# kawshik8/GAN-Image-Captioning

Hardware: AMD Instinct MI355X
Metric: captions/sec (G+D train step) (higher is better)
Workload: dtype bf16; 1 GPU; cfg2: adversarial G+D step, batch 64/GPU, 224x224 images, caption len 20, V=10000, E=H=512, 1-layer LSTM G, CNN-seq D (R=64,F=900), ResNet-50-shaped encoder, --conditional-gan 1; global_batch=64, caption_len=20, image_size=224, vocab=10000, conditional_gan=1, encoder=resnet50, step_impl=fused, parallelism=dp1

## Files before the change

### gan-image-captioning_amd/csrc/decoder.hip

```cpp
#include <stdlib.h>

#include "../../include/gicap.h"
#include "decoder_step.h"
#include "kernels.h"

namespace gic {
namespace {

__device__ __forceinline__ float sigmoidf_(float x) { return 1.f / (1.f + expf(-x)); }

template <typename TA>
__global__ void lstm_pointwise_fwd_kernel(const float* __restrict__ gpre, const float* __restrict__ c_prev,
                                          float* __restrict__ gates, float* __restrict__ c_new,
                                          TA* __restrict__ h_next, long ld_next,
                                          TA* __restrict__ h_up, long ld_up,
                                          TA* __restrict__ h_out, long ld_out,
                                          int B, int H) {
  const int idx = blockIdx.x * blockDim.x + threadIdx.x;
  if (idx >= B * H) return;
  const int b = idx / H, j = idx % H;
  const float* g = gpre + (long)b * 4 * H;
  const float i_ = sigmoidf_(g[j]);
  const float f_ = sigmoidf_(g[H + j]);
  const float g_ = tanhf(g[2 * H + j]);
// ... 240 lines not shown
    *(uint4*)dv[i] = *(const uint4*)(dp + o);
  }
  float s = 0.f;
#pragma unroll
  for (int i = 0; i < NCH; ++i) {
    if (threadIdx.x + 256 * i < nch) {
#pragma unroll
      for (int k = 0; k < VN; ++k) s += to_f32<TA>(pv[i][k]) * to_f32<TA>(dv[i][k]);
    }
  }
  s = block_sum(s, red);
#pragma unroll
  for (int i = 0; i < NCH; ++i) {
    const int c = threadIdx.x + 256 * i;
    if (c < nch) {
      TA ov[VN];
#pragma unroll
      for (int k = 0; k < VN; ++k) ov[k] = from_f32<TA>(temperature * to_f32<TA>(pv[i][k]) * (to_f32<TA>(dv[i][k]) - s));
      *(uint4*)(dl + row * V + (long)c * VN) = *(const uint4*)ov;
    }
  }
}

template <typename TA>
__global__ void build_wcat_kernel(const float* __restrict__ w_ih, const float* __restrict__ w_hh,
                                  const float* __restrict__ b_ih, const float* __restrict__ b_hh,
                                  TA* __restrict__ wcat, float* __restrict__ bsum, int rows, int din, int hid) {
  const long ld = din + hid;
  const long total = (long)rows * ld;
  for (long i = (long)blockIdx.x * blockDim.x + threadIdx.x; i < total; i += (long)gridDim.x * blockDim.x) {
    const long r = i / ld;
    const int c = (int)(i % ld);
    const float v = c < din ? w_ih[r * din + c] : w_hh[r * hid + (c - din)];
    wcat[i] = from_f32<TA>(v);
    if (c == 0) bsum[r] = b_ih[r] + b_hh[r];
  }
}

template <int PB>
__global__ void rollout_join_kernel(const unsigned char* __restrict__ src_xh, unsigned char* __restrict__ dst_xh, long rowbytes,
                                    const float* __restrict__ src_c, float* __restrict__ dst_c, int H, long r0, long r1, int srcB) {
  typedef typename std::conditional<PB == 16, uint4, typename std::conditional<PB == 4, uint32_t, uint16_t>::type>::type piece_t;
  const long pieces = rowbytes / PB;
  const long total = (r1 - r0) * pieces;
  for (long i = (long)blockIdx.x * blockDim.x + threadIdx.x; i < total; i += (long)gridDim.x * blockDim.x) {
    const long r = r0 + i / pieces, p = i % pieces;
    *(piece_t*)(dst_xh + r * rowbytes + p * PB) = *(const piece_t*)(src_xh + (r % srcB) * rowbytes + p * PB);
  }
  const long totc = (r1 - r0) * H;
  for (long i = (long)blockIdx.x * blockDim.x + threadIdx.x; i < totc; i += (long)gridDim.x * blockDim.x) {
    const long r = r0 + i / H;
    dst_c[r * H + i % H] = src_c[(r % srcB) * H + i % H];
  }
}

template <typename TA>
__global__ __launch_bounds__(256) void rollout_pick_kernel(const unsigned long long* __restrict__ rowkey, int64_t* __restrict__ ids, long ids_stride,
                                                           const float* __restrict__ embed, TA* __restrict__ x_next, long ld_x, int rows, int V,
                                                           int E, const int64_t* __restrict__ force_ids, const int32_t* __restrict__ force_len,
// ... 4 lines not shown
  if (force_ids && (!force_len || t < force_len[b])) id = (int)force_ids[(long)b * ids_stride];
  id = id < 0 ? 0 : (id >= V ? V - 1 : id);
  if (lane == 0) ids[(long)b * ids_stride] = id;
  if (x_next)
    for (int e = lane; e < E; e += 64) x_next[(long)b * ld_x + e] = from_f32<TA>(embed[(long)id * E + e]);
}

struct Ctx {
  int B, L, V, E, H, NL, dt;
  int din(int l) const { return l == 0 ? E : H; }
  long ldx(int l) const { return (long)din(l) + H; }
  size_t asz() const { return (size_t)dtype_size(dt); }
};

int check_dims(const gic_decoder_dims* d, Ctx& c) {
  GIC_CHECK_ARG(d, "decoder: null dims");
  GIC_CHECK_ARG(d->B > 0 && d->L > 0 && d->V > 1 && d->E > 0 && d->H > 0, "decoder: bad dims");
  GIC_CHECK_ARG(d->NL >= 1 && d->NL <= GIC_MAX_LAYERS, "decoder: gen_num_layers must be 1..%d", GIC_MAX_LAYERS);
  GIC_CHECK_ARG(d->dtype == DT_F32 || d->dtype == DT_BF16, "decoder: bad dtype");
  c = Ctx{d->B, d->L, d->V, d->E, d->H, d->NL, d->dtype};
  return GIC_OK;
}

int init_slot0(const Ctx& c, const gic_decoder_state* st, const float* features, const gic_decoder_sample_opts* opt, hipStream_t stream) {
  const int B = c.B, E = c.E, H = c.H;
  for (int l = 0; l < c.NL; ++l) {
    if (opt && opt->h0) {
      if (l > 0) GIC_PROPAGATE(fill_zero(st->xh[l], (size_t)B * c.ldx(l) * c.asz(), stream));
      GIC_PROPAGATE(cast2d(opt->h0 + (long)l * B * H, DT_F32, H, (char*)st->xh[l] + (size_t)c.din(l) * c.asz(), c.dt, c.ldx(l), B, H, stream));
    } else {
      GIC_PROPAGATE(fill_zero(st->xh[l], (size_t)B * c.ldx(l) * c.asz(), stream));
    }
    if (opt && opt->c0) GIC_PROPAGATE(cast2d(opt->c0 + (long)l * B * H, DT_F32, H, st->c[l], DT_F32, H, B, H, stream));
    else GIC_PROPAGATE(fill_zero(st->c[l], (size_t)B * H * sizeof(float), stream));
  }
  return cast2d(features, DT_F32, E, st->xh[0], c.dt, c.ldx(0), B, E, stream);
}

template <typename TA>
int sample_fwd_fused(const Ctx& c, const gic_decoder_params* P, const gic_decoder_shadow* S, const gic_decoder_state* st,
                     const float* noise_u, uint64_t seed, float temperature, int pretrain, void* out, int64_t* ids,
                     const gic_decoder_sample_opts* opt, hipStream_t stream) {
  const int B = c.B, L = c.L, V = c.V, H = c.H, NL = c.NL;
  const int nblk = cdiv(V, kVocabTile);
  const long per = (long)L * B * nblk;
  float* part_m = st->part;
  float* part_s = st->part + per;
  unsigned long long* rowkey = (unsigned long long*)(st->part + ((2 * per + 1) & ~1l));
  GIC_PROPAGATE(fill_zero(rowkey, (size_t)L * B * sizeof(unsigned long long), stream));
  const bool keep = !(opt && opt->no_state);
  for (int t = 0; t < L; ++t) {
    for (int l = 0; l < NL; ++l) {
      const long ld = c.ldx(l);
      LstmStepArgs a;
      a.xh_t = (TA*)st->xh[l] + (long)t * B * ld;
      a.xh_next = (TA*)st->xh[l] + (long)(t + 1) * B * ld;
      a.wcat = S->wcat[l]; a.bsum = S->bsum[l];
      a.c_prev = st->c[l] + (long)t * B * H; a.c_new = st->c[l] + (long)(t + 1) * B * H;
      a.gates = keep ? st->gates[l] + (long)t * B * 4 * H : nullptr;
      if (l + 1 < NL) { a.h_up = (TA*)st->xh[l + 1] + (long)t * B * c.ldx(l + 1); a.ld_up = c.ldx(l + 1); }
      if (l + 1 == NL && st->hout) { a.h_out = (TA*)st->hout + (long)t * H; a.ld_out = (long)L * H; }
      a.B = B; a.H = H; a.din = c.din(l); a.ldx = ld;
      if (l == 0 && t > 0) {
        a.gather = 1; a.embed = P->embed; a.V = V;
        a.rowkey = rowkey + (long)(t - 1) * B;
        if (opt && opt->force_ids) { a.force_ids = opt->force_ids; a.force_stride = L; a.force_len = opt->force_len; }
        a.tprev = t - 1;
      }
      GIC_PROPAGATE(lstm_step(a, c.dt, stream));
    }
    VocabStepArgs v;
    const int l = NL - 1;
// ... 1 lines not shown
    v.wout = S->wout; v.bias = P->b_out;
    v.u = noise_u ? noise_u + (long)t * B * V : nullptr;
    v.seed = seed; v.rng_stream = (uint64_t)t; v.temperature = temperature; v.pretrain = pretrain;
    if (opt && opt->dev_scalars) { v.t_dev = &opt->dev_scalars->temperature; v.seed_dev = &opt->dev_scalars->seed[opt->seed_slot]; }
    v.out = out ? (void*)((TA*)out + (long)t * V) : nullptr; v.out_stride = (long)L * V;
    v.part_m = part_m + (long)t * B * nblk; v.part_s = part_s + (long)t * B * nblk; v.rowkey = rowkey + (long)t * B;
    v.nblk = nblk; v.B = B; v.V = V; v.H = H;
    GIC_PROPAGATE(vocab_step(v, c.dt, stream));
  }
  SampleFinishArgs f;
  f.part_m = part_m; f.part_s = part_s; f.rowkey = rowkey; f.nblk = nblk; f.B = B; f.L = L; f.V = V; f.E = c.E;
  f.pretrain = pretrain; f.out = out; f.ids = ids;
  if (opt && opt->force_ids) { f.force_ids = opt->force_ids; f.force_len = opt->force_len; }
  if (keep) { f.embed = P->embed; f.xh0 = st->xh[0]; f.ldx0 = c.ldx(0); }
  return sample_finish(f, c.dt, stream);
}

template <typename TA>
int sample_fwd_t(const Ctx& c, const gic_decoder_params* P, const gic_decoder_shadow* S, const gic_decoder_state* st,
                 const float* features, const float* noise_u, uint64_t seed, float temperature, int pretrain,
                 void* out, int64_t* ids, const gic_decoder_sample_opts* opt, hipStream_t stream) {
  const int B = c.B, L = c.L, V = c.V, E = c.E, H = c.H, NL = c.NL;
  const int pw_grid = cdiv((long)B * H, 256);
  GIC_PROPAGATE(init_slot0(c, st, features, opt, stream));
  if (st->part && B <= decoder_step_max_rows() && !(opt && opt->resume_from) && decoder_step_supported(c.dt, V, E, H, NL))
    return sample_fwd_fused<TA>(c, P, S, st, noise_u, seed, temperature, pretrain, out, ids, opt, stream);
  if (opt && opt->dev_scalars) {
    set_last_error("decoder_sample_fwd: device-resident step scalars need the fused step kernels (state->part, B <= %d, V %% 4 == 0, E, H %% 8 == 0)",
                   decoder_step_max_rows());
    return GIC_ERR_UNSUPPORTED;
  }
  GIC_CHECK_ARG(st->logits && st->gpre, "decoder_sample_fwd: the unfused path needs state->logits and state->gpre");
  const bool keep = !(opt && opt->no_state);
  const int64_t* f_ids = opt ? opt->force_ids : nullptr;
  const int32_t* f_len = opt ? opt->force_len : nullptr;
  const int32_t* act = (opt && opt->resume_from) ? opt->host_active_rows : nullptr;
  if (act) GIC_PROPAGATE(hipMemcpyAsync(ids, f_ids, (size_t)B * L * sizeof(int64_t), hipMemcpyDeviceToDevice, stream) == hipSuccess ? GIC_OK : GIC_ERR_LAUNCH);
  unsigned long long* rowkeys = nullptr;
  if (!out && !pretrain && c.dt == DT_BF16 && V % 4 == 0 && (long)L * 8 <= (long)V * 4 && ((uintptr_t)st->logits & 7) == 0) {
    rowkeys = (unsigned long long*)st->logits;
    GIC_PROPAGATE(fill_zero(rowkeys, (size_t)L * B * sizeof(unsigned long long), stream));
  }

  for (int t = 0; t < L; ++t) {
    const int M = act ? act[t] : B;
    if (act) {
      const int M_prev = t > 0 ? act[t - 1] : 0;
      if (M > M_prev) {
        for (int l = 0; l < NL; ++l) {
          const long rowbytes = c.ldx(l) * (long)c.asz();
          GIC_PROPAGATE(rollout_join((const unsigned char*)opt->resume_from->xh[l] + (size_t)t * opt->resume_B * rowbytes,
                                     (unsigned char*)st->xh[l] + (size_t)t * B * rowbytes, rowbytes,
                                     (const float*)(opt->resume_from->c[l] + (long)t * opt->resume_B * H), st->c[l] + (long)t * B * H, H, M_prev, M,
                                     opt->resume_B, stream));
        }
      }
      if (M == 0) continue;
    }
    const int pw_grid_t = cdiv((long)M * H, 256);
    for (int l = 0; l < NL; ++l) {
      const long ld = c.ldx(l);
      TA* xh_t = (TA*)st->xh[l] + (long)t * B * ld;
      TA* xh_n = (TA*)st->xh[l] + (long)(t + 1) * B * ld;
      GemmDesc g;
      g.A = xh_t; g.lda = ld; g.B = S->wcat[l]; g.ldb = ld; g.C = st->gpre; g.ldc = 4 * H;
// ... 385 lines not shown
int gumbel_softmax_rows(int dt, float* logits, const float* u, uint64_t seed, uint64_t rng_stream, float temperature, int pretrain, void* out,
                        long rows, int V, hipStream_t stream) {
  if (dt == DT_F32)
    hipLaunchKernelGGL((gumbel_softmax_argmax_kernel<float>), dim3((unsigned)rows), dim3(256), 0, stream, logits, u, seed, rng_stream, temperature,
                       pretrain, (float*)out, (long)V, (int64_t*)nullptr, (long)1, (const float*)nullptr, (float*)nullptr, (long)0, V, 0,
                       (const int64_t*)nullptr, (const int32_t*)nullptr, 0);
  else
    hipLaunchKernelGGL((gumbel_softmax_argmax_kernel<bf16_t>), dim3((unsigned)rows), dim3(256), 0, stream, logits, u, seed, rng_stream,
                       temperature, pretrain, (bf16_t*)out, (long)V, (int64_t*)nullptr, (long)1, (const float*)nullptr, (bf16_t*)nullptr, (long)0,
                       V, 0, (const int64_t*)nullptr, (const int32_t*)nullptr, 0);
  GIC_CHECK_LAUNCH("gumbel_softmax (teacher forced)");
  return GIC_OK;
}

namespace {

template <typename TA>
int forward_tf_t(const Ctx& c, const gic_decoder_params* P, const gic_decoder_shadow* S, const gic_decoder_state* st,
                 const float* features, const int64_t* caps, const int32_t* lengths, int Tmax, const float* noise_u, uint64_t seed,
                 float temperature, int pretrain, float* logits_ws, void* out, float* h_n, float* c_n, hipStream_t stream,
                 const gic_sched_sample_opts* ss = nullptr) {
  const int B = c.B, T = c.L, V = c.V, E = c.E, H = c.H, NL = c.NL;
  const int pw_grid = cdiv((long)B * H, 256);
  for (int l = 0; l < NL; ++l) {
    GIC_PROPAGATE(fill_zero(st->xh[l], (size_t)B * c.ldx(l) * c.asz(), stream));
    GIC_PROPAGATE(fill_zero(st->c[l], (size_t)B * H * sizeof(float), stream));
  }
  GIC_PROPAGATE(cast2d(features, DT_F32, E, st->xh[0], c.dt, c.ldx(0), B, E, stream));
  GIC_PROPAGATE(embed_rows_tf(c.dt, P->embed, caps, st->xh[0], c.ldx(0), B, T - 1, E, V, stream));
  const bool ss_fused = ss && ss_fused_logits(c.dt, B, V, E, H, NL);
  if (ss) GIC_PROPAGATE(ss_tail(caps, ss->inputs, ss->replaced, B, T - 1, Tmax - 1, stream));
  for (int t = 0; t < Tmax; ++t) {
    for (int l = 0; l < NL; ++l) {
      const long ld = c.ldx(l);
      TA* xh_t = (TA*)st->xh[l] + (long)t * B * ld;
      TA* xh_n = (TA*)st->xh[l] + (long)(t + 1) * B * ld;
      GemmDesc g;
      g.A = xh_t; g.lda = ld; g.B = S->wcat[l]; g.ldb = ld; g.C = st->gpre; g.ldc = 4 * H;
      g.M = B; g.N = 4 * H; g.K = (int)ld; g.in_dtype = c.dt; g.out_dtype = DT_F32; g.bias = S->bsum[l];
      g.no_split = ss != nullptr;
      GIC_PROPAGATE(gemm(g, stream));
      TA* h_up = (l + 1 < NL) ? (TA*)st->xh[l + 1] + (long)t * B * c.ldx(l + 1) : nullptr;
      TA* h_out = (l + 1 == NL) ? (TA*)st->hout + (long)t * H : nullptr;
      hipLaunchKernelGGL((lstm_pointwise_tf_kernel<TA>), dim3(pw_grid), dim3(256), 0, stream, (const float*)st->gpre,
                         (const float*)(st->c[l] + (long)t * B * H), (const TA*)(xh_t + c.din(l)), ld,
                         st->c[l] + (long)(t + 1) * B * H, xh_n + c.din(l), ld, h_up, h_up ? c.ldx(l + 1) : 0, h_out, (long)Tmax * H,
                         lengths, t, B, H, st->gates[l] ? st->gates[l] + (long)t * B * 4 * H : nullptr);
      GIC_CHECK_LAUNCH("lstm_pointwise_tf");
    }
    if (ss) {
      GIC_PROPAGATE(ss_step_logits(c.dt, st->hout, t, Tmax, S->wout, P->b_out, logits_ws, B, V, H, ss_fused, stream));
// ... 140 lines not shown
}

int gic_decoder_bwd_ws_bytes(const gic_decoder_dims* dims, uint64_t* out) {
  Ctx c;
  GIC_PROPAGATE(check_dims(dims, c));
  GIC_CHECK_ARG(out, "decoder_bwd_ws_bytes: null out");
  const uint64_t B = c.B, L = c.L, H = c.H, a = c.asz();
  out[0] = B * L * (uint64_t)c.V * a;
  out[1] = B * L * H * 4;
  for (int l = 0; l < GIC_MAX_LAYERS; ++l) {
    const bool on = l < c.NL;
    out[2 + l] = on ? L * B * 4 * H * a : 0;
    out[2 + GIC_MAX_LAYERS + l] = on ? (L + 1) * B * (uint64_t)c.ldx(l) * 4 : 0;
    out[2 + 2 * GIC_MAX_LAYERS + l] = on ? B * H * 4 : 0;
  }
  return GIC_OK;
}

int gic_decoder_prepare(const gic_decoder_dims* dims, const gic_decoder_params* P, const gic_decoder_shadow* S, void* stream_) {
  Ctx c;
  GIC_PROPAGATE(check_dims(dims, c));
  GIC_CHECK_ARG(P && S, "decoder_prepare: null struct");
  hipStream_t stream = (hipStream_t)stream_;
  for (int l = 0; l < c.NL; ++l) {
    GIC_CHECK_ARG(P->w_ih[l] && P->w_hh[l] && P->b_ih[l] && P->b_hh[l] && S->wcat[l] && S->bsum[l], "decoder_prepare: null layer %d", l);
    const long total = (long)4 * c.H * c.ldx(l);
    const int grid = (int)((total + 255) / 256 > 2048 ? 2048 : (total + 255) / 256);
    if (c.dt == DT_F32)
      hipLaunchKernelGGL((build_wcat_kernel<float>), dim3(grid), dim3(256), 0, stream, P->w_ih[l], P->w_hh[l], P->b_ih[l],
                         P->b_hh[l], (float*)S->wcat[l], S->bsum[l], 4 * c.H, c.din(l), c.H);
    else
      hipLaunchKernelGGL((build_wcat_kernel<bf16_t>), dim3(grid), dim3(256), 0, stream, P->w_ih[l], P->w_hh[l], P->b_ih[l],
                         P->b_hh[l], (bf16_t*)S->wcat[l], S->bsum[l], 4 * c.H, c.din(l), c.H);
    GIC_CHECK_LAUNCH("build_wcat");
    if (S->wcat_t[l]) GIC_PROPAGATE(transpose2d(S->wcat[l], S->wcat_t[l], c.dt, 4 * c.H, c.ldx(l), stream));
  }
  GIC_CHECK_ARG(P->w_out && S->wout, "decoder_prepare: null w_out");
  if ((const void*)S->wout != (const void*)P->w_out)
    GIC_PROPAGATE(cast2d(P->w_out, DT_F32, c.H, S->wout, c.dt, c.H, c.V, c.H, stream));
  return GIC_OK;
}

int gic_decoder_sample_fwd(const gic_decoder_dims* dims, const gic_decoder_params* P, const gic_decoder_shadow* S,
                           const gic_decoder_state* st, const float* features, const float* noise_u, uint64_t seed,
                           float temperature, int pretrain, void* out, int64_t* ids, const gic_decoder_sample_opts* opt,
                           void* stream) {
  Ctx c;
  GIC_PROPAGATE(check_dims(dims, c));
  GIC_CHECK_ARG(P && S && st && features && ids, "decoder_sample_fwd: null argument");
  const bool keep = !(opt && opt->no_state);
  GIC_CHECK_ARG(!keep || (st->hout && out), "decoder_sample_fwd: out / state->hout may be NULL only for a stateless roll-out (opts->no_state)");
  GIC_CHECK_ARG(!(opt && opt->force_len && !opt->force_ids), "decoder_sample_fwd: force_len without force_ids");
  GIC_CHECK_ARG(!(opt && opt->dev_scalars) || (opt->seed_slot >= 0 && opt->seed_slot < GIC_STEP_SEEDS), "decoder_sample_fwd: seed_slot out of range");
  if (opt && opt->resume_from) {
    GIC_CHECK_ARG(opt->force_ids && opt->force_len && opt->host_active_rows && opt->resume_B > 0 && opt->no_state,
                  "decoder_sample_fwd: resumed roll-outs need force_ids, force_len, host_active_rows, resume_B and no_state");
    for (int l = 0; l < c.NL; ++l) GIC_CHECK_ARG(opt->resume_from->xh[l] && opt->resume_from->c[l], "decoder_sample_fwd: resume_from lacks layer %d state", l);
    for (int t = 0; t < c.L; ++t)
      GIC_CHECK_ARG(opt->host_active_rows[t] >= (t ? opt->host_active_rows[t - 1] : 0) && opt->host_active_rows[t] <= c.B,
                    "decoder_sample_fwd: host_active_rows must be non-decreasing and <= B");
    GIC_CHECK_ARG(opt->host_active_rows[0] == 0, "decoder_sample_fwd: resumed rows have a prefix of at least one token");
  }
  for (int l = 0; l < c.NL; ++l)
// ... 31 lines not shown
```

### gan-image-captioning_amd/csrc/disc.hip

```cpp
#include <stdlib.h>
#include "../../include/gicap.h"
#include "kernels.h"
#include "gemm_device.h"

namespace gic {
namespace {

constexpr int kMaxTaps = 32;
constexpr int kOutDim = 100;
constexpr int kOutPad = 104;

struct ConvMeta {
  int nconv, F, Fp, s;
  int fsize[GIC_MAX_CONVS], nfilt[GIC_MAX_CONVS], foff[GIC_MAX_CONVS];
  const float* w[GIC_MAX_CONVS];
  const float* b[GIC_MAX_CONVS];
  float* dw[GIC_MAX_CONVS];
  float* db[GIC_MAX_CONVS];
};

__device__ __forceinline__ int conv_of(const ConvMeta& cm, int col) {
  int k = 0;
  while (k + 1 < cm.nconv && col >= cm.foff[k + 1]) ++k;
  return k;
// ... 877 lines not shown
  out[5] = MR * Fp * a;
  out[6] = MR * kOutDim * 4;
  return GIC_OK;
}

int gic_disc_bwd_ws_bytes(const gic_disc_dims* dims, uint64_t* out) {
  DCtx c;
  GIC_PROPAGATE(make_ctx(dims, nullptr, nullptr, c));
  GIC_CHECK_ARG(out, "disc_bwd_ws_bytes: null out");
  const uint64_t a = dtype_size(c.dt), MR = c.rowsBR, Fp = c.Fp;
  out[0] = MR * kOutPad * a;
  out[1] = MR * Fp * a;
  out[2] = MR * Fp * 4;
  out[3] = MR * Fp * 4;
  out[4] = (uint64_t)c.rowsBL * c.De * a;
  return GIC_OK;
}

int gic_disc_prepare(const gic_disc_dims* dims, const gic_disc_params* P, const gic_disc_shadow* S, void* stream_) {
  DCtx c;
  GIC_PROPAGATE(make_ctx(dims, P, nullptr, c));
  GIC_CHECK_ARG(P && S && P->emb && P->hw_w && P->f2o_w && S->emb && S->hw_w && S->f2o_w, "disc_prepare: null pointer");
  hipStream_t stream = (hipStream_t)stream_;
  if ((const void*)S->emb != (const void*)P->emb)
    GIC_PROPAGATE(cast2d(P->emb, DT_F32, c.V, S->emb, c.dt, c.V, c.De, c.V, stream));
  const size_t a = dtype_size(c.dt);
  GIC_PROPAGATE(fill_zero(S->hw_w, (size_t)c.Fp * c.Fp * a, stream));
  GIC_PROPAGATE(cast2d(P->hw_w, DT_F32, c.F, S->hw_w, c.dt, c.Fp, c.F, c.F, stream));
  if (S->hw_w_t) GIC_PROPAGATE(transpose2d(S->hw_w, S->hw_w_t, c.dt, c.Fp, c.Fp, stream));
  GIC_PROPAGATE(fill_zero(S->f2o_w, (size_t)kOutPad * c.Fp * a, stream));
  GIC_PROPAGATE(cast2d(P->f2o_w, DT_F32, c.F, S->f2o_w, c.dt, c.Fp, kOutDim, c.F, stream));
  return GIC_OK;
}

int gic_disc_fwd(const gic_disc_dims* dims, const gic_disc_params* P, const gic_disc_shadow* S, const gic_disc_state* st,
                 const void* inp_soft, int64_t ld_inp, const int64_t* inp_ids, int train, const uint8_t* keep_mask,
                 uint64_t seed, float* logits, const gic_step_scalars* dev_scalars, int seed_slot, void* stream) {
  DCtx c;
  GIC_CHECK_ARG(!dev_scalars || (seed_slot >= 0 && seed_slot < GIC_STEP_SEEDS), "disc_fwd: seed_slot out of range");
  const uint64_t* seed_dev = dev_scalars ? &dev_scalars->seed[seed_slot] : nullptr;
  GIC_PROPAGATE(make_ctx(dims, P, nullptr, c));
  GIC_CHECK_ARG(P && S && st && logits, "disc_fwd: null argument");
  GIC_CHECK_ARG((inp_soft != nullptr) != (inp_ids != nullptr), "disc_fwd: pass exactly one of inp_soft / inp_ids");
  GIC_CHECK_ARG(!inp_soft || ld_inp >= c.V, "disc_fwd: ld_inp < V");
  GIC_CHECK_ARG(st->emb && st->pooled && st->ydrop && st->feat && (!train || (st->keep && st->argmax && st->hpre)), "disc_fwd: null state buffer");
  GIC_CHECK_ARG(P->emb && P->hw_b && P->f2o_b && P->o2l_w && P->o2l_b && S->emb && S->hw_w && S->f2o_w, "disc_fwd: null parameter");
  if (c.dt == DT_F32)
    return disc_fwd_t<float>(c, P, S, st, inp_soft, ld_inp, inp_ids, train, keep_mask, seed, seed_dev, logits, (hipStream_t)stream);
  return disc_fwd_t<bf16_t>(c, P, S, st, inp_soft, ld_inp, inp_ids, train, keep_mask, seed, seed_dev, logits, (hipStream_t)stream);
}

int gic_disc_fwd_redrop(const gic_disc_dims* dims, const gic_disc_params* P, const gic_disc_shadow* S, const gic_disc_state* src,
                        const gic_disc_state* dst, int train, const uint8_t* keep_mask, uint64_t seed, float* logits,
                        const gic_step_scalars* dev_scalars, int seed_slot, void* stream) {
  DCtx c;
// ... 50 lines not shown
```

### gan-image-captioning_amd/csrc/kernels.h

```cpp
#pragma once
#include "common.h"
#include "gemm.h"

struct gic_sched_sample_opts;

namespace gic {

int cast2d(const void* src, int src_dtype, long lds, void* dst, int dst_dtype, long ldd, long rows, long cols,
           hipStream_t stream);
int colsum(const void* A, int dtype, long lda, long rows, long cols, float* out, float* out2, int accumulate,
           hipStream_t stream, float* scratch = nullptr, long scratch_floats = 0);
int embedding_fwd(const float* weight, const int64_t* ids, float* out, long n, int V, int E, hipStream_t stream);
int embedding_bwd(const float* d_out, const int64_t* ids, float* d_weight, long n, int V, int E, int zero_first,
                  hipStream_t stream);
int fill_zero(void* p, size_t bytes, hipStream_t stream);
int transpose2d(const void* src, void* dst, int dtype, long rows, long cols, hipStream_t stream);

int decoder_output_bwd(int dt, int B, int L, int V, int H, const void* probs, const void* d_out, float temperature, const float* t_dev, int pretrain,
                       void* dlogits_ws, const void* wout, const void* hout, float* dhout, float* d_wout, float* d_bout, hipStream_t stream);
int lstm_pointwise_fwd(int dt, const float* gpre, const float* c_prev, float* c_new, void* h_next, long ld_next, void* h_up, long ld_up,
                       int rows, int H, hipStream_t stream);
int rollout_join(const unsigned char* src_xh, unsigned char* dst_xh, long rowbytes, const float* src_c, float* dst_c, int H, long r0, long r1,
                 int srcB, hipStream_t stream);
int rollout_pick(int dt, const unsigned long long* rowkey, int64_t* ids, long ids_stride, const float* embed, void* x_next, long ld_x, int rows,
                 int V, int E, const int64_t* force_ids, const int32_t* force_len, int t, hipStream_t stream);
int rollout_argmax(int dt, float* logits, const float* u, uint64_t seed, uint64_t rng_stream, float temperature, int pretrain, void* out,
                   long out_stride, int64_t* ids, long ids_stride, const float* embed, void* x_next, long ld_x, int rows, int V, int E,
                   const int64_t* force_ids, const int32_t* force_len, int t, hipStream_t stream);
int det_mode();
int det_scatter(const void* src, int dt, long ld, long row_off, const int64_t* ids, int B, long s_b, long s_t, long n, float* dst,
                long d_id, long d_e, int E, int V, hipStream_t stream);
int embed_rows_tf(int dt, const float* embed, const int64_t* caps, void* xh0, long ld, int B, int Tm1, int E, int V, hipStream_t stream);
int zero_past_length(float* dhout, const int32_t* lengths, int B, int Tmax, int H, hipStream_t stream);
int gumbel_softmax_rows(int dt, float* logits, const float* u, uint64_t seed, uint64_t rng_stream, float temperature, int pretrain, void* out,
                        long rows, int V, hipStream_t stream);
int embed_scatter_time(const float* dx, long ld, const int64_t* ids, float* d_embed, int B, int L, int E, int V, hipStream_t stream, long ids_stride = 0);

struct SsPickArgs {
  const float* logits = nullptr; long ld_logits = 0;
// ... 24 lines not shown
```

### gan-image-captioning_amd/csrc/util.hip

```cpp
#include <stdarg.h>
#include <stdio.h>

#include "../../include/gicap.h"
#include "kernels.h"

namespace gic {

static thread_local char g_last_error[512] = "";

void set_last_error(const char* fmt, ...) {
  va_list ap;
  va_start(ap, fmt);
  vsnprintf(g_last_error, sizeof(g_last_error), fmt, ap);
  va_end(ap);
}

static thread_local bool g_route_only = false;
static thread_local char g_route[kRouteLen] = "";
bool route_only() { return g_route_only; }
char* route_line() { return g_route; }

namespace {

template <typename TA>
// ... 119 lines not shown

__global__ void embedding_fwd_kernel(const float* __restrict__ w, const int64_t* __restrict__ ids, float* __restrict__ out,
                                     long n, int V, int E) {
  const long total = n * E;
  for (long i = (long)blockIdx.x * blockDim.x + threadIdx.x; i < total; i += (long)gridDim.x * blockDim.x) {
    const long r = i / E;
    const int e = (int)(i % E);
    long id = ids[r];
    id = id < 0 ? 0 : (id >= V ? V - 1 : id);
    out[i] = w[id * E + e];
  }
}

__global__ void embedding_bwd_kernel(const float* __restrict__ dout, const int64_t* __restrict__ ids,
                                     float* __restrict__ dw, long n, int V, int E) {
  const long total = n * E;
  for (long i = (long)blockIdx.x * blockDim.x + threadIdx.x; i < total; i += (long)gridDim.x * blockDim.x) {
    const long r = i / E;
    const int e = (int)(i % E);
    long id = ids[r];
    id = id < 0 ? 0 : (id >= V ? V - 1 : id);
    atomicAdd(&dw[id * E + e], dout[i]);
  }
}

inline int grid_for(long total, int block = 256, int cap = 2048) {
  long g = (total + block - 1) / block;
  return (int)(g < 1 ? 1 : (g > cap ? cap : g));
}

}

int transpose2d(const void* src, void* dst, int dtype, long rows, long cols, hipStream_t stream) {
  GIC_CHECK_ARG(src && dst && rows > 0 && cols > 0, "transpose2d: bad argument");
  const dim3 tg((unsigned)cdiv(cols, 32), (unsigned)cdiv(rows, 32));
  if (dtype == DT_F32)
    hipLaunchKernelGGL((transpose2d_kernel<float>), tg, dim3(256), 0, stream, (const float*)src, (float*)dst, (int)rows, (int)cols);
  else
    hipLaunchKernelGGL((transpose2d_kernel<bf16_t>), tg, dim3(256), 0, stream, (const bf16_t*)src, (bf16_t*)dst, (int)rows, (int)cols);
  GIC_CHECK_LAUNCH("transpose2d");
  return GIC_OK;
}

int fill_zero(void* p, size_t bytes, hipStream_t stream) {
  if (bytes == 0) return GIC_OK;
  hipError_t e = hipMemsetAsync(p, 0, bytes, stream);
// ... 7 lines not shown
int cast2d(const void* src, int sdt, long lds, void* dst, int ddt, long ldd, long rows, long cols, hipStream_t stream) {
  GIC_CHECK_ARG(src && dst, "cast2d: null pointer");
  if (rows * cols == 0) return GIC_OK;
  const int g = grid_for(rows * cols);
  if (sdt == DT_F32 && ddt == DT_F32)
    hipLaunchKernelGGL((cast2d_kernel<float, float>), dim3(g), dim3(256), 0, stream, (const float*)src, lds, (float*)dst, ldd, rows, cols);
  else if (sdt == DT_F32 && ddt == DT_BF16 && cols % 8 == 0 && lds % 4 == 0 && ldd % 8 == 0 && ((((uintptr_t)src) | ((uintptr_t)dst)) & 15) == 0)
    hipLaunchKernelGGL(cast2d_f32_bf16_vec_kernel, dim3(grid_for(rows * cols / 16)), dim3(256), 0, stream, (const float*)src, lds, (bf16_t*)dst, ldd,
                       rows, cols);
  else if (sdt == DT_F32 && ddt == DT_BF16)
    hipLaunchKernelGGL((cast2d_kernel<float, bf16_t>), dim3(g), dim3(256), 0, stream, (const float*)src, lds, (bf16_t*)dst, ldd, rows, cols);
  else if (sdt == DT_BF16 && ddt == DT_F32)
    hipLaunchKernelGGL((cast2d_kernel<bf16_t, float>), dim3(g), dim3(256), 0, stream, (const bf16_t*)src, lds, (float*)dst, ldd, rows, cols);
  else if (sdt == DT_BF16 && ddt == DT_BF16)
    hipLaunchKernelGGL((cast2d_kernel<bf16_t, bf16_t>), dim3(g), dim3(256), 0, stream, (const bf16_t*)src, lds, (bf16_t*)dst, ldd, rows, cols);
  else {
    set_last_error("cast2d: bad dtypes %d -> %d", sdt, ddt);
    return GIC_ERR_UNSUPPORTED;
  }
  GIC_CHECK_LAUNCH("cast2d");
  return GIC_OK;
}

static int colsum_fold(const float* part, int gy, long cols, float* out, float* out2, hipStream_t stream) {
  hipLaunchKernelGGL(colsum_fold_kernel, dim3((unsigned)cdiv(cols, 256)), dim3(256), 0, stream, part, gy, cols, out, out2);
  GIC_CHECK_LAUNCH("colsum_fold");
  return GIC_OK;
}

static int det_colsum_rows(int gy, int accumulate, long cols, long scratch_floats, bool* slab) {
  int g = gy < 64 ? gy : 64;
  if (g > 1 && scratch_floats / cols >= 2) {
    if (g > scratch_floats / cols) g = (int)(scratch_floats / cols);
    *slab = true;
    return g;
  }
  *slab = false;
  const int cap = accumulate ? 1 : 2;
  return gy < cap ? gy : cap;
}

int colsum(const void* A, int dtype, long lda, long rows, long cols, float* out, float* out2, int accumulate,
           hipStream_t stream, float* scratch, long scratch_floats) {
  GIC_CHECK_ARG(A && out, "colsum: null pointer");
  if (cols == 0) return GIC_OK;
  if (!accumulate) {
// ... 106 lines not shown
```

Before: 26690 captions/s.

## Fuse weight-image prep and rollout slot-0 init into single kernels

Replaces the per-layer build_wcat, transpose, fill_zero and cast launches in decoder_prepare and disc_prepare with one weight_images kernel. Each block either builds a tiled weight image, writing the transposed copy through shared memory, or casts a chunk of the output/embedding weights. Separately, the slot-0 initialisation of xh/c plus zeroing of the row keys becomes one rollout_slot0_kernel instead of several fill_zero/cast2d launches. The aim is to cut launch count and redundant memory passes per train step, at the cost of more complex indexing and alignment-dependent paths.

```diff
diff --git a/gan-image-captioning_amd/csrc/decoder.hip b/gan-image-captioning_amd/csrc/decoder.hip
--- a/gan-image-captioning_amd/csrc/decoder.hip
+++ b/gan-image-captioning_amd/csrc/decoder.hip
@@ -286,19 +286,53 @@
   }
 }
 
-template <typename TA>
-__global__ void build_wcat_kernel(const float* __restrict__ w_ih, const float* __restrict__ w_hh,
-                                  const float* __restrict__ b_ih, const float* __restrict__ b_hh,
-                                  TA* __restrict__ wcat, float* __restrict__ bsum, int rows, int din, int hid) {
-  const long ld = din + hid;
-  const long total = (long)rows * ld;
-  for (long i = (long)blockIdx.x * blockDim.x + threadIdx.x; i < total; i += (long)gridDim.x * blockDim.x) {
-    const long r = i / ld;
-    const int c = (int)(i % ld);
-    const float v = c < din ? w_ih[r * din + c] : w_hh[r * hid + (c - din)];
-    wcat[i] = from_f32<TA>(v);
-    if (c == 0) bsum[r] = b_ih[r] + b_hh[r];
-  }
+struct Slot0Args {
+  void* xh[GIC_MAX_LAYERS]; float* c[GIC_MAX_LAYERS];
+  const float* features; const float* h0; const float* c0;
+  unsigned long long* keys; long nkeys;
+  int B, E, H, vec;
+};
+
+template <typename TA>
+__global__ __launch_bounds__(256) void rollout_slot0_kernel(const Slot0Args A) {
+  const int b = blockIdx.x, l = blockIdx.y, t = threadIdx.x;
+  void* xh_l = A.xh[0]; float* c_l = A.c[0];
+#pragma unroll
+  for (int q = 1; q < GIC_MAX_LAYERS; ++q)
+    if (l == q) { xh_l = A.xh[q]; c_l = A.c[q]; }
+  const int H = A.H, din = l == 0 ? A.E : H, ld = din + H;
+  TA* xrow = (TA*)xh_l + (long)b * ld;
+  float* crow = c_l + (long)b * H;
+  const float* xsrc = l == 0 ? A.features + (long)b * A.E : nullptr;
+  const float* hsrc = A.h0 ? A.h0 + ((long)l * A.B + b) * H : nullptr;
+  const float* csrc = A.c0 ? A.c0 + ((long)l * A.B + b) * H : nullptr;
+  if (A.vec) {
+    const int npx = ld >> 3, npc = H >> 2;
+    for (int p = t; p < npx || p < npc; p += 256) {
+      const int col = p * 8;
+      const float* s = nullptr;
+      if (p < npx) s = col < din ? (xsrc ? xsrc + col : nullptr) : (hsrc ? hsrc + (col - din) : nullptr);
+      const float* sp = s ? s : A.features;
+      const f32x4 v0 = *(const f32x4*)sp, v1 = *(const f32x4*)(sp + 4);
+      const bool cs = csrc && p < npc;
+      const f32x4 vc = *(const f32x4*)(cs ? csrc + p * 4 : A.features);
+      if (p < npx) {
+        float f[8];
+#pragma unroll
+        for (int k = 0; k < 4; ++k) { f[k] = s ? v0[k] : 0.f; f[4 + k] = s ? v1[k] : 0.f; }
+        store8_from_f32<TA>(xrow + col, f);
+      }
+      if (p < npc) *(f32x4*)(crow + p * 4) = cs ? vc : f32x4{0.f, 0.f, 0.f, 0.f};
+    }
+  } else {
+    for (int col = t; col < ld; col += 256) {
+      const float* s = col < din ? (xsrc ? xsrc + col : nullptr) : (hsrc ? hsrc + (col - din) : nullptr);
+      xrow[col] = from_f32<TA>(s ? *s : 0.f);
+    }
+    for (int j = t; j < H; j += 256) crow[j] = csrc ? csrc[j] : 0.f;
+  }
+  const long stride = (long)gridDim.x * gridDim.y * 256;
+  for (long i = ((long)l * gridDim.x + b) * 256 + t; i < A.nkeys; i += stride) A.keys[i] = 0ull;
 }
 
 template <int PB>
@@ -349,19 +383,30 @@
   return GIC_OK;
 }
 
-int init_slot0(const Ctx& c, const gic_decoder_state* st, const float* features, const gic_decoder_sample_opts* opt, hipStream_t stream) {
-  const int B = c.B, E = c.E, H = c.H;
-  for (int l = 0; l < c.NL; ++l) {
-    if (opt && opt->h0) {
-      if (l > 0) GIC_PROPAGATE(fill_zero(st->xh[l], (size_t)B * c.ldx(l) * c.asz(), stream));
-      GIC_PROPAGATE(cast2d(opt->h0 + (long)l * B * H, DT_F32, H, (char*)st->xh[l] + (size_t)c.din(l) * c.asz(), c.dt, c.ldx(l), B, H, stream));
-    } else {
-      GIC_PROPAGATE(fill_zero(st->xh[l], (size_t)B * c.ldx(l) * c.asz(), stream));
-    }
-    if (opt && opt->c0) GIC_PROPAGATE(cast2d(opt->c0 + (long)l * B * H, DT_F32, H, st->c[l], DT_F32, H, B, H, stream));
-    else GIC_PROPAGATE(fill_zero(st->c[l], (size_t)B * H * sizeof(float), stream));
-  }
-  return cast2d(features, DT_F32, E, st->xh[0], c.dt, c.ldx(0), B, E, stream);
+static bool slot0_in_pieces(const Ctx& c, const Slot0Args& a) {
+  uintptr_t bits = (uintptr_t)a.features | (uintptr_t)a.h0 | (uintptr_t)a.c0;
+  for (int l = 0; l < c.NL; ++l) bits |= (uintptr_t)a.xh[l] | (uintptr_t)a.c[l];
+  return c.E % 8 == 0 && c.H % 8 == 0 && (bits & 15) == 0;
+}
+
+int init_slot0(const Ctx& c, const gic_decoder_state* st, const float* features, const gic_decoder_sample_opts* opt, unsigned long long* keys,
+               long nkeys, hipStream_t stream) {
+  Slot0Args a = {};
+  for (int l = 0; l < c.NL; ++l) { a.xh[l] = st->xh[l]; a.c[l] = st->c[l]; }
+  a.features = features; a.h0 = opt ? opt->h0 : nullptr; a.c0 = opt ? opt->c0 : nullptr;
+  a.keys = keys; a.nkeys = keys ? nkeys : 0;
+  a.B = c.B; a.E = c.E; a.H = c.H; a.vec = slot0_in_pieces(c, a) ? 1 : 0;
+  if (c.dt == DT_F32)
+    hipLaunchKernelGGL((rollout_slot0_kernel<float>), dim3((unsigned)c.B, (unsigned)c.NL), dim3(256), 0, stream, a);
+  else
+    hipLaunchKernelGGL((rollout_slot0_kernel<bf16_t>), dim3((unsigned)c.B, (unsigned)c.NL), dim3(256), 0, stream, a);
+  GIC_CHECK_LAUNCH("rollout_slot0");
+  return GIC_OK;
+}
+
+unsigned long long* fused_rowkeys(const Ctx& c, const gic_decoder_state* st) {
+  const long per = (long)c.L * c.B * cdiv(c.V, kVocabTile);
+  return (unsigned long long*)(st->part + ((2 * per + 1) & ~1l));
 }
 
 template <typename TA>
@@ -373,8 +418,7 @@
   const long per = (long)L * B * nblk;
   float* part_m = st->part;
   float* part_s = st->part + per;
-  unsigned long long* rowkey = (unsigned long long*)(st->part + ((2 * per + 1) & ~1l));
-  GIC_PROPAGATE(fill_zero(rowkey, (size_t)L * B * sizeof(unsigned long long), stream));
+  unsigned long long* rowkey = fused_rowkeys(c, st);
   const bool keep = !(opt && opt->no_state);
   for (int t = 0; t < L; ++t) {
     for (int l = 0; l < NL; ++l) {
@@ -422,9 +466,10 @@
                  void* out, int64_t* ids, const gic_decoder_sample_opts* opt, hipStream_t stream) {
   const int B = c.B, L = c.L, V = c.V, E = c.E, H = c.H, NL = c.NL;
   const int pw_grid = cdiv((long)B * H, 256);
-  GIC_PROPAGATE(init_slot0(c, st, features, opt, stream));
-  if (st->part && B <= decoder_step_max_rows() && !(opt && opt->resume_from) && decoder_step_supported(c.dt, V, E, H, NL))
+  if (st->part && B <= decoder_step_max_rows() && !(opt && opt->resume_from) && decoder_step_supported(c.dt, V, E, H, NL)) {
+    GIC_PROPAGATE(init_slot0(c, st, features, opt, fused_rowkeys(c, st), (long)L * B, stream));
     return sample_fwd_fused<TA>(c, P, S, st, noise_u, seed, temperature, pretrain, out, ids, opt, stream);
+  }
   if (opt && opt->dev_scalars) {
     set_last_error("decoder_sample_fwd: device-resident step scalars need the fused step kernels (state->part, B <= %d, V %% 4 == 0, E, H %% 8 == 0)",
                    decoder_step_max_rows());
@@ -437,10 +482,9 @@
   const int32_t* act = (opt && opt->resume_from) ? opt->host_active_rows : nullptr;
   if (act) GIC_PROPAGATE(hipMemcpyAsync(ids, f_ids, (size_t)B * L * sizeof(int64_t), hipMemcpyDeviceToDevice, stream) == hipSuccess ? GIC_OK : GIC_ERR_LAUNCH);
   unsigned long long* rowkeys = nullptr;
-  if (!out && !pretrain && c.dt == DT_BF16 && V % 4 == 0 && (long)L * 8 <= (long)V * 4 && ((uintptr_t)st->logits & 7) == 0) {
+  if (!out && !pretrain && c.dt == DT_BF16 && V % 4 == 0 && (long)L * 8 <= (long)V * 4 && ((uintptr_t)st->logits & 7) == 0)
     rowkeys = (unsigned long long*)st->logits;
-    GIC_PROPAGATE(fill_zero(rowkeys, (size_t)L * B * sizeof(unsigned long long), stream));
-  }
+  GIC_PROPAGATE(init_slot0(c, st, features, opt, rowkeys, (long)L * B, stream));
 
   for (int t = 0; t < L; ++t) {
     const int M = act ? act[t] : B;
@@ -872,11 +916,7 @@
                  const gic_sched_sample_opts* ss = nullptr) {
   const int B = c.B, T = c.L, V = c.V, E = c.E, H = c.H, NL = c.NL;
   const int pw_grid = cdiv((long)B * H, 256);
-  for (int l = 0; l < NL; ++l) {
-    GIC_PROPAGATE(fill_zero(st->xh[l], (size_t)B * c.ldx(l) * c.asz(), stream));
-    GIC_PROPAGATE(fill_zero(st->c[l], (size_t)B * H * sizeof(float), stream));
-  }
-  GIC_PROPAGATE(cast2d(features, DT_F32, E, st->xh[0], c.dt, c.ldx(0), B, E, stream));
+  GIC_PROPAGATE(init_slot0(c, st, features, nullptr, nullptr, 0, stream));
   GIC_PROPAGATE(embed_rows_tf(c.dt, P->embed, caps, st->xh[0], c.ldx(0), B, T - 1, E, V, stream));
   const bool ss_fused = ss && ss_fused_logits(c.dt, B, V, E, H, NL);
   if (ss) GIC_PROPAGATE(ss_tail(caps, ss->inputs, ss->replaced, B, T - 1, Tmax - 1, stream));
@@ -1063,23 +1103,19 @@
   GIC_PROPAGATE(check_dims(dims, c));
   GIC_CHECK_ARG(P && S, "decoder_prepare: null struct");
   hipStream_t stream = (hipStream_t)stream_;
+  static_assert(GIC_MAX_LAYERS <= ImageJobs::kMaxTile, "one tile job per layer");
+  ImageJobs J;
   for (int l = 0; l < c.NL; ++l) {
     GIC_CHECK_ARG(P->w_ih[l] && P->w_hh[l] && P->b_ih[l] && P->b_hh[l] && S->wcat[l] && S->bsum[l], "decoder_prepare: null layer %d", l);
-    const long total = (long)4 * c.H * c.ldx(l);
-    const int grid = (int)((total + 255) / 256 > 2048 ? 2048 : (total + 255) / 256);
-    if (c.dt == DT_F32)
-      hipLaunchKernelGGL((build_wcat_kernel<float>), dim3(grid), dim3(256), 0, stream, P->w_ih[l], P->w_hh[l], P->b_ih[l],
-                         P->b_hh[l], (float*)S->wcat[l], S->bsum[l], 4 * c.H, c.din(l), c.H);
-    else
-      hipLaunchKernelGGL((build_wcat_kernel<bf16_t>), dim3(grid), dim3(256), 0, stream, P->w_ih[l], P->w_hh[l], P->b_ih[l],
-                         P->b_hh[l], (bf16_t*)S->wcat[l], S->bsum[l], 4 * c.H, c.din(l), c.H);
-    GIC_CHECK_LAUNCH("build_wcat");
-    if (S->wcat_t[l]) GIC_PROPAGATE(transpose2d(S->wcat[l], S->wcat_t[l], c.dt, 4 * c.H, c.ldx(l), stream));
+    ImageTileJob& j = J.tile[J.ntile++];
+    j.a = P->w_ih[l]; j.lda = c.din(l); j.b = P->w_hh[l]; j.ldb = c.H;
+    j.split = c.din(l); j.SR = j.IR = 4 * c.H; j.SC = j.IC = (int)c.ldx(l);
+    j.img = S->wcat[l]; j.img_t = S->wcat_t[l];
+    j.bias_a = P->b_ih[l]; j.bias_b = P->b_hh[l]; j.bsum = S->bsum[l];
   }
   GIC_CHECK_ARG(P->w_out && S->wout, "decoder_prepare: null w_out");
-  if ((const void*)S->wout != (const void*)P->w_out)
-    GIC_PROPAGATE(cast2d(P->w_out, DT_F32, c.H, S->wout, c.dt, c.H, c.V, c.H, stream));
-  return GIC_OK;
+  if ((const void*)S->wout != (const void*)P->w_out) { J.cast_src = P->w_out; J.cast_dst = S->wout; J.cast_n = (long)c.V * c.H; }
+  return weight_images(J, c.dt, stream);
 }
 
 int gic_decoder_sample_fwd(const gic_decoder_dims* dims, const gic_decoder_params* P, const gic_decoder_shadow* S,
diff --git a/gan-image-captioning_amd/csrc/disc.hip b/gan-image-captioning_amd/csrc/disc.hip
--- a/gan-image-captioning_amd/csrc/disc.hip
+++ b/gan-image-captioning_amd/csrc/disc.hip
@@ -923,15 +923,15 @@
   GIC_PROPAGATE(make_ctx(dims, P, nullptr, c));
   GIC_CHECK_ARG(P && S && P->emb && P->hw_w && P->f2o_w && S->emb && S->hw_w && S->f2o_w, "disc_prepare: null pointer");
   hipStream_t stream = (hipStream_t)stream_;
-  if ((const void*)S->emb != (const void*)P->emb)
-    GIC_PROPAGATE(cast2d(P->emb, DT_F32, c.V, S->emb, c.dt, c.V, c.De, c.V, stream));
-  const size_t a = dtype_size(c.dt);
-  GIC_PROPAGATE(fill_zero(S->hw_w, (size_t)c.Fp * c.Fp * a, stream));
-  GIC_PROPAGATE(cast2d(P->hw_w, DT_F32, c.F, S->hw_w, c.dt, c.Fp, c.F, c.F, stream));
-  if (S->hw_w_t) GIC_PROPAGATE(transpose2d(S->hw_w, S->hw_w_t, c.dt, c.Fp, c.Fp, stream));
-  GIC_PROPAGATE(fill_zero(S->f2o_w, (size_t)kOutPad * c.Fp * a, stream));
-  GIC_PROPAGATE(cast2d(P->f2o_w, DT_F32, c.F, S->f2o_w, c.dt, c.Fp, kOutDim, c.F, stream));
-  return GIC_OK;
+  ImageJobs J;
+  ImageTileJob& hw = J.tile[J.ntile++];
+  hw.a = P->hw_w; hw.lda = c.F; hw.split = hw.SC = hw.SR = c.F; hw.IR = hw.IC = c.Fp;
+  hw.img = S->hw_w; hw.img_t = S->hw_w_t;
+  ImageTileJob& fo = J.tile[J.ntile++];
+  fo.a = P->f2o_w; fo.lda = c.F; fo.split = fo.SC = c.F; fo.SR = kOutDim; fo.IR = kOutPad; fo.IC = c.Fp;
+  fo.img = S->f2o_w;
+  if ((const void*)S->emb != (const void*)P->emb) { J.cast_src = P->emb; J.cast_dst = S->emb; J.cast_n = (long)c.De * c.V; }
+  return weight_images(J, c.dt, stream);
 }
 
 int gic_disc_fwd(const gic_disc_dims* dims, const gic_disc_params* P, const gic_disc_shadow* S, const gic_disc_state* st,
diff --git a/gan-image-captioning_amd/csrc/kernels.h b/gan-image-captioning_amd/csrc/kernels.h
--- a/gan-image-captioning_amd/csrc/kernels.h
+++ b/gan-image-captioning_amd/csrc/kernels.h
@@ -15,6 +15,27 @@
                   hipStream_t stream);
 int fill_zero(void* p, size_t bytes, hipStream_t stream);
 int transpose2d(const void* src, void* dst, int dtype, long rows, long cols, hipStream_t stream);
+
+struct ImageTileJob {
+  const float* a = nullptr; const float* b = nullptr; long lda = 0, ldb = 0;
+  int split = 0, SR = 0, SC = 0, IR = 0, IC = 0;
+  void* img = nullptr; void* img_t = nullptr;
+  const float* bias_a = nullptr; const float* bias_b = nullptr; float* bsum = nullptr;
+};
+struct ImageJobs {
+  static constexpr int kMaxTile = 4;
+  ImageTileJob tile[kMaxTile];
+  int ntile = 0;
+  const float* cast_src = nullptr; void* cast_dst = nullptr; long cast_n = 0;
+};
+int weight_images(const ImageJobs& jobs, int dtype, hipStream_t stream);
+template <typename T> __device__ __forceinline__ void store8_from_f32(T* p, const float (&v)[8]) {
+  alignas(16) T o[8];
+#pragma unroll
+  for (int k = 0; k < 8; ++k) o[k] = from_f32<T>(v[k]);
+#pragma unroll
+  for (int q = 0; q < (int)(8 * sizeof(T) / 16); ++q) ((uint4*)p)[q] = ((const uint4*)o)[q];
+}
 
 int decoder_output_bwd(int dt, int B, int L, int V, int H, const void* probs, const void* d_out, float temperature, const float* t_dev, int pretrain,
                        void* dlogits_ws, const void* wout, const void* hout, float* dhout, float* d_wout, float* d_bout, hipStream_t stream);
diff --git a/gan-image-captioning_amd/csrc/util.hip b/gan-image-captioning_amd/csrc/util.hip
--- a/gan-image-captioning_amd/csrc/util.hip
+++ b/gan-image-captioning_amd/csrc/util.hip
@@ -165,6 +165,137 @@
     id = id < 0 ? 0 : (id >= V ? V - 1 : id);
     atomicAdd(&dw[id * E + e], dout[i]);
   }
+}
+
+constexpr int kImgTile = 64, kImgCastBlock = 8192;
+struct ImageArgs {
+  ImageTileJob tile[ImageJobs::kMaxTile];
+  int blk0[ImageJobs::kMaxTile + 1];
+  int tiles_c[ImageJobs::kMaxTile];
+  int tile_vec[ImageJobs::kMaxTile];
+  int ntile, cast_vec;
+  const float* cast_src; void* cast_dst; long cast_n;
+};
+
+template <typename TA>
+__device__ __forceinline__ void image_tile_pieces(const ImageTileJob& j, const int r0, const int c0, float (*tile)[kImgTile + 1]) {
+  const int cg = threadIdx.x & 7, rw = threadIdx.x >> 3;
+  f32x4 v[2][2];
+#pragma unroll
+  for (int i = 0; i < 2; ++i)
+#pragma unroll
+    for (int p = 0; p < 2; ++p) {
+      const int r = r0 + rw + 32 * i, c = c0 + cg * 8 + 4 * p;
+      const int rr = r < j.SR ? r : j.SR - 1, cc = c < j.SC ? c : 0;
+      v[i][p] = *(const f32x4*)(cc < j.split ? j.a + (long)rr * j.lda + cc : j.b + (long)rr * j.ldb + (cc - j.split));
+    }
+#pragma unroll
+  for (int i = 0; i < 2; ++i) {
+    const int r = r0 + rw + 32 * i, c = c0 + cg * 8;
+    float f[8];
+#pragma unroll
+    for (int k = 0; k < 8; ++k) {
+      f[k] = (r < j.SR && c + (k & 4) < j.SC) ? v[i][k >> 2][k & 3] : 0.f;
+      tile[rw + 32 * i][cg * 8 + k] = f[k];
+    }
+    if (r < j.IR && c < j.IC) store8_from_f32<TA>((TA*)j.img + (long)r * j.IC + c, f);
+  }
+  if (!j.img_t) return;
+  __syncthreads();
+#pragma unroll
+  for (int i = 0; i < 2; ++i) {
+    const int oc = c0 + rw + 32 * i, orow = r0 + cg * 8;
+    float f[8];
+#pragma unroll
+    for (int k = 0; k < 8; ++k) f[k] = tile[cg * 8 + k][rw + 32 * i];
+    if (oc < j.IC && orow < j.IR) store8_from_f32<TA>((TA*)j.img_t + (long)oc * j.IR + orow, f);
+  }
+}
+
+template <typename TA>
+__device__ __forceinline__ void image_tile_scalar(const ImageTileJob& j, const int r0, const int c0, float (*tile)[kImgTile + 1]) {
+  const int cx = threadIdx.x & 63, ry = threadIdx.x >> 6;
+  float f[16];
+  const int c = c0 + cx, cc = c < j.SC ? c : 0;
+#pragma unroll
+  for (int i = 0; i < 16; ++i) {
+    const int r = r0 + ry + 4 * i, rr = r < j.SR ? r : j.SR - 1;
+    f[i] = cc < j.split ? j.a[(long)rr * j.lda + cc] : j.b[(long)rr * j.ldb + (cc - j.split)];
+  }
+#pragma unroll
+  for (int i = 0; i < 16; ++i) {
+    const int r = r0 + ry + 4 * i;
+    if (!(r < j.SR && c < j.SC)) f[i] = 0.f;
+    tile[ry + 4 * i][cx] = f[i];
+    if (r < j.IR && c < j.IC) ((TA*)j.img)[(long)r * j.IC + c] = from_f32<TA>(f[i]);
+  }
+  if (!j.img_t) return;
+  __syncthreads();
+#pragma unroll
+  for (int i = 0; i < 16; ++i) {
+    const int oc = c0 + ry + 4 * i, orow = r0 + cx;
+    if (oc < j.IC && orow < j.IR) ((TA*)j.img_t)[(long)oc * j.IR + orow] = from_f32<TA>(tile[cx][ry + 4 * i]);
+  }
+}
+
+template <typename TA>
+__device__ __forceinline__ void image_cast_block(const float* __restrict__ src, TA* __restrict__ dst, const long n, const long e0, const int vec) {
+  const int t = threadIdx.x;
+  if (vec) {
+    const long np = n >> 3, p0 = e0 >> 3;
+    f32x4 v[4][2];
+#pragma unroll
+    for (int u = 0; u < 4; ++u) {
+      const long p = p0 + t + 256 * u, pp = p < np ? p : 0;
+      v[u][0] = *(const f32x4*)(src + pp * 8);
+      v[u][1] = *(const f32x4*)(src + pp * 8 + 4);
+    }
+#pragma unroll
+    for (int u = 0; u < 4; ++u) {
+      const long p = p0 + t + 256 * u;
+      float f[8];
+#pragma unroll
+      for (int k = 0; k < 8; ++k) f[k] = v[u][k >> 2][k & 3];
+      if (p < np) store8_from_f32<TA>(dst + p * 8, f);
+    }
+    if (e0 == 0 && np * 8 + t < n) dst[np * 8 + t] = from_f32<TA>(src[np * 8 + t]);
+    return;
+  }
+#pragma unroll 1
+  for (int u0 = 0; u0 < kImgCastBlock / 256; u0 += 8) {
+    float f[8];
+#pragma unroll
+    for (int u = 0; u < 8; ++u) {
+      const long e = e0 + t + 256 * (u0 + u);
+      f[u] = src[e < n ? e : 0];
+    }
+#pragma unroll
+    for (int u = 0; u < 8; ++u) {
+      const long e = e0 + t + 256 * (u0 + u);
+      if (e < n) dst[e] = from_f32<TA>(f[u]);
+    }
+  }
+}
+
+template <typename TA>
+__global__ __launch_bounds__(256) void weight_images_kernel(const ImageArgs A) {
+  __shared__ float tile[kImgTile][kImgTile + 1];
+  const int b = blockIdx.x;
+  if (b >= A.blk0[A.ntile]) {
+    image_cast_block<TA>(A.cast_src, (TA*)A.cast_dst, A.cast_n, (long)(b - A.blk0[A.ntile]) * kImgCastBlock, A.cast_vec);
+    return;
+  }
+  ImageTileJob j = A.tile[0];
+  int first = A.blk0[0], tiles_c = A.tiles_c[0], vec = A.tile_vec[0];
+#pragma unroll
+  for (int q = 1; q < ImageJobs::kMaxTile; ++q)
+    if (q < A.ntile && b >= A.blk0[q]) { j = A.tile[q]; first = A.blk0[q]; tiles_c = A.tiles_c[q]; vec = A.tile_vec[q]; }
+  const int ti = b - first, tr = ti / tiles_c, tc = ti - tr * tiles_c;
+  const int r0 = tr * kImgTile, c0 = tc * kImgTile;
+  if (vec) image_tile_pieces<TA>(j, r0, c0, tile);
+  else image_tile_scalar<TA>(j, r0, c0, tile);
+  if (j.bsum && tc == 0 && threadIdx.x < kImgTile && r0 + (int)threadIdx.x < j.SR)
+    j.bsum[r0 + threadIdx.x] = j.bias_a[r0 + threadIdx.x] + j.bias_b[r0 + threadIdx.x];
 }
 
 inline int grid_for(long total, int block = 256, int cap = 2048) {
@@ -218,6 +349,47 @@
   return GIC_OK;
 }
 
+static bool aligned16(const void* p) { return ((uintptr_t)p & 15) == 0; }
+static bool image_tile_in_pieces(const ImageTileJob& j) {
+  const bool two = j.split < j.SC;
+  return j.split % 4 == 0 && j.SC % 4 == 0 && j.lda % 4 == 0 && (!two || j.ldb % 4 == 0) && j.IC % 8 == 0 && (!j.img_t || j.IR % 8 == 0) &&
+         aligned16(j.a) && (!two || aligned16(j.b)) && aligned16(j.img) && aligned16(j.img_t);
+}
+static bool image_cast_in_pieces(const ImageJobs& J) { return aligned16(J.cast_src) && aligned16(J.cast_dst); }
+
+int weight_images(const ImageJobs& J, int dt, hipStream_t stream) {
+  GIC_CHECK_ARG(J.ntile >= 0 && J.ntile <= ImageJobs::kMaxTile && (dt == DT_F32 || dt == DT_BF16), "weight_images: bad job list");
+  ImageArgs A = {};
+  long nb = 0;
+  for (int l = 0; l < J.ntile; ++l) {
+    const ImageTileJob& j = J.tile[l];
+    GIC_CHECK_ARG(j.a && j.img && j.split > 0 && j.split <= j.SC && (j.split == j.SC || j.b) && j.SR > 0 && j.SR <= j.IR && j.SC <= j.IC &&
+                      j.lda >= j.split && (j.split == j.SC || j.ldb >= j.SC - j.split) && (!j.bsum || (j.bias_a && j.bias_b)),
+                  "weight_images: bad tile job %d", l);
+    A.tile[l] = j;
+    A.blk0[l] = (int)nb;
+    A.tiles_c[l] = cdiv(j.IC, kImgTile);
+    A.tile_vec[l] = image_tile_in_pieces(j) ? 1 : 0;
+    nb += (long)cdiv(j.IR, kImgTile) * A.tiles_c[l];
+  }
+  A.ntile = J.ntile;
+  A.blk0[J.ntile] = (int)nb;
+  if (J.cast_n > 0) {
+    GIC_CHECK_ARG(J.cast_src && J.cast_dst, "weight_images: null cast job");
+    A.cast_src = J.cast_src; A.cast_dst = J.cast_dst; A.cast_n = J.cast_n;
+    A.cast_vec = image_cast_in_pieces(J) ? 1 : 0;
+    nb += cdiv(J.cast_n, kImgCastBlock);
+  }
+  if (nb == 0) return GIC_OK;
+  GIC_CHECK_ARG(nb < (1l << 31), "weight_images: too many blocks");
+  if (dt == DT_F32)
+    hipLaunchKernelGGL((weight_images_kernel<float>), dim3((unsigned)nb), dim3(256), 0, stream, A);
+  else
+    hipLaunchKernelGGL((weight_images_kernel<bf16_t>), dim3((unsigned)nb), dim3(256), 0, stream, A);
+  GIC_CHECK_LAUNCH("weight_images");
+  return GIC_OK;
+}
+
 static int colsum_fold(const float* part, int gy, long cols, float* out, float* out2, hipStream_t stream) {
   hipLaunchKernelGGL(colsum_fold_kernel, dim3((unsigned)cdiv(cols, 256)), dim3(256), 0, stream, part, gy, cols, out, out2);
   GIC_CHECK_LAUNCH("colsum_fold");
```

New measurement: 26690 captions/s (median of 3 runs). No clear change (-0.0%).
